# qiqiqicheng/news-recommendation-tc

Hardware: AMD Instinct MI355X
Metric: recalled pairs/sec (YouTubeDNN top-30) + DIN scored pairs/sec, 1/2/4/8 MI355X (higher is better)
Workload: dtype fp16

## Files before the change

### news-recommendation-tc_amd/csrc/ip_topk.hip

```cpp
#include "nrk_common.h"

#include <float.h>
#include <math.h>
#include <stdlib.h>

#include <algorithm>
#include <atomic>
#include <type_traits>
#include <utility>

namespace nrk {

typedef float f32x16 __attribute__((ext_vector_type(16)));
typedef _Float16 f16x8 __attribute__((ext_vector_type(8)));
typedef unsigned u32x4 __attribute__((ext_vector_type(4)));
typedef float f32x4 __attribute__((ext_vector_type(4)));

constexpr int IP_KFAST = 128;
constexpr int IP_KMAX = 2048;
constexpr int SCAN_TILE = 8192;
constexpr int SCAN_TB128 = 4;
__host__ __device__ constexpr int scan_tb(int dp) {
    return dp == 128 ? SCAN_TB128 : (64 * dp >= SCAN_TILE ? 1 : SCAN_TILE / (64 * dp));
}
constexpr int IP_SEL = 512;
constexpr int IP_BQ = 288;
constexpr int IP_KRING = 256;
constexpr size_t CATALOG_HDR = 256;

__host__ __device__ static inline int pad_dim(int d) {
    return d <= 16 ? 16 : d <= 32 ? 32 : d <= 64 ? 64 : d <= 128 ? 128 : 256;
}
__host__ __device__ static inline int64_t n_blocks_of(int64_t n_items) { return (n_items + 31) / 32; }

struct CatalogHdr {
    float max_norm;
    float max_abs;
    float scale;
    int32_t dim;
    int32_t dp;
    float max_dnorm;
};

__device__ __forceinline__ float pow2_scale(float maxabs) {
    if (!(maxabs > 0.0f)) return 1.0f;
    int e;
    (void)frexpf(maxabs, &e);
    return ldexpf(1.0f, 14 - e);
}

// ... 360 lines not shown
}
__device__ __forceinline__ void pf_wait(u32x4 (&cur)[2]) {
    asm volatile("s_waitcnt lgkmcnt(0)" : "+v"(cur[0]), "+v"(cur[1])::"memory");
}
template <int OFF>
__device__ __forceinline__ void pf_issue_at(uint32_t base, u32x4 (&af)[2]) {
    asm volatile("ds_read_b128 %0, %2 offset:%3\n\tds_read_b128 %1, %2 offset:%4"
                 : "=&v"(af[0]), "=&v"(af[1])
                 : "v"(base), "n"(OFF), "n"(OFF + 1024)
                 : "memory");
}
template <int OFF>
__device__ __forceinline__ void pf_wait_issue_at(u32x4 (&cur)[2], uint32_t base, u32x4 (&nxt)[2]) {
    asm volatile("s_waitcnt lgkmcnt(0)\n\tds_read_b128 %0, %4 offset:%5\n\tds_read_b128 %1, %4 offset:%6"
                 : "=&v"(nxt[0]), "=&v"(nxt[1]), "+v"(cur[0]), "+v"(cur[1])
                 : "v"(base), "n"(OFF), "n"(OFF + 1024)
                 : "memory");
}

template <int DP, int NW, int NSL, int UG, int MT>
__global__ __launch_bounds__(NW * 64, 2) void ip_scan_kernel(
    const float* __restrict__ users, int n_users, const uint8_t* __restrict__ catalog, int n_items, int dim, int k,
    int m2, uint2* __restrict__ app, int32_t* __restrict__ acnt, float4* __restrict__ uinfo, int tile_lo,
    int tile_hi, int n_pre, int pstride, float* __restrict__ bnd, int bnd_m) {
    constexpr int DS = DP / 16;
    constexpr int BLOCK_BYTES = 64 * DP;
    constexpr int TB = scan_tb(DP);
    constexpr int TILE_BYTES = TB * BLOCK_BYTES;
    constexpr int LPT = TILE_BYTES / (NW * 1024);
    static_assert(LPT >= 1 && LPT * NW * 1024 == TILE_BYTES, "tile split");
    static_assert(NSL >= 2, "ring");
    __shared__ __attribute__((aligned(16))) uint8_t smem[NSL * TILE_BYTES];

    const int tid = threadIdx.x;
    const int wave = tid >> 6, lane = tid & 63, h = lane >> 5, q = lane & 31;
    const int ub = blockIdx.x;
    const int ubase = ub * (NW * 32 * UG) + wave * (32 * UG);
#if NRK_SCAN_STAMP
    uint64_t sstp[8] = {0, 0, 0, 0, 0, 0, 0, 0};
    uint64_t t_prev = 0;
#endif

    const int nblk = (n_items + 31) >> 5;
    const int ntile = tile_hi;
    const CatalogHdr* hdr = reinterpret_cast<const CatalogHdr*>(catalog + (size_t)nblk * BLOCK_BYTES);
    const float vmax = hdr->max_norm, sv_scale = hdr->scale, dvmax = hdr->max_dnorm;
    const int jk = (k + 1) / 2 - 1;

    f16x8 ufrag[UG][DS];
    float eps_s[UG], tau[UG];
    float t[UG][MT];
    bool live[UG];
#pragma unroll
    for (int g = 0; g < UG; ++g) {
        const int user = ubase + g * 32 + q;
        float eps, scl;
        scan_user_setup<DS>(users, n_users, dim, user, h, vmax, dvmax, sv_scale, ufrag[g], eps, scl, live[g]);
        eps_s[g] = eps * scl;
        if (h == 0 && user < n_users) uinfo[user] = make_float4(-INFINITY, eps_s[g], scl, eps);
        tau[g] = live[g] ? -FLT_MAX : INFINITY;
#pragma unroll
        for (int i = 0; i < MT; ++i) t[g][i] = (live[g] && i >= MT - 1 - jk) ? -INFINITY : INFINITY;
    }
    uint2* const wapp = app + (size_t)(ub * (NW * 32 * UG) + __builtin_amdgcn_readfirstlane(wave) * (32 * UG)) *
                                  2 * (size_t)m2;
    uint32_t pos[UG], lim[UG];
#pragma unroll
    for (int g = 0; g < UG; ++g) {
        pos[g] = (uint32_t)((g * 32 + q) * 2 + h) * (uint32_t)m2;
        lim[g] = pos[g] + (uint32_t)m2 - 1u;
    }
    auto slot = [&](uint32_t x, int g) -> uint32_t { return min(x, lim[g]); };
    auto app_store_if = [&](uint64_t m, uint32_t e, uint2 v) { app_store_masked(m, wapp, e << 3, v); };

    const uint32_t lds_base = (uint32_t)(uintptr_t)(const __attribute__((address_space(3))) uint8_t*)(smem);
    const int body_bytes = nblk * BLOCK_BYTES;
    const int tail_blk = n_items >> 5;
    const int last_tile = (nblk - 1) / TB;
    auto issue_tile = [&](int tt, int sl) {
        uint8_t* slot = smem + sl * TILE_BYTES;
        const uint32_t ttc = (uint32_t)min(tt, last_tile);
#pragma unroll
// ... 256 lines not shown
            if (h == 0) reinterpret_cast<float*>(uinfo + user)[0] = live[g] ? lb : -INFINITY;
        }
    }
    if constexpr (MT <= 32) {
        if (bnd != nullptr) {
#pragma unroll
            for (int g = 0; g < UG; ++g)
                list_bound_out<MT>(t[g], live[g], h, ubase + g * 32 + q, n_users, jk, bnd, bnd_m, uinfo);
        }
    }
}

constexpr int SCAN_WS_NB = 2;
constexpr int SCAN_WS_TPS = 2;
constexpr int SCAN_WS_PRIO = 2;
constexpr int SCAN_WS_INSP = 8, SCAN_WS_SHARD_INSP = 4;
static_assert((SCAN_WS_INSP & (SCAN_WS_INSP - 1)) == 0 && SCAN_WS_INSP >= SCAN_WS_TPS &&
                  (SCAN_WS_SHARD_INSP & (SCAN_WS_SHARD_INSP - 1)) == 0 && SCAN_WS_SHARD_INSP >= SCAN_WS_TPS,
              "insert periods: powers of two >= the two tiles of a step");
template <int DP, int NSL, int MT>
__global__ __launch_bounds__(64 * 4 * (1 + SCAN_WS_NB), 1) void ip_scan_ws_kernel(
    const float* __restrict__ users, int n_users, const uint8_t* __restrict__ catalog, int n_items, int dim, int k,
    int m2, uint2* __restrict__ app, int32_t* __restrict__ acnt, float4* __restrict__ uinfo, int tile_lo,
    int tile_hi, int n_pre, int pstride, float* __restrict__ bnd, int bnd_m, int insp) {
    constexpr int NPW = 4, UG = 8, NB = SCAN_WS_NB, UGB = UG / NB, DS = DP / 16;
    constexpr int BLOCK_BYTES = 64 * DP;
    constexpr int TB = scan_tb(DP);
    constexpr int TILE_BYTES = TB * BLOCK_BYTES;
    constexpr int NPC = TILE_BYTES / 1024;
    static_assert(TB == 4 && DS == 2 && NPC == 8 && UGB == 4, "WS scan: 8-KB tiles of four blocks at DP = 32");
    constexpr int TPS = SCAN_WS_TPS, NMX = 2 * TPS, LPW = NPC / NPW, DAHEAD = NSL / TPS - 1;
    static_assert(NSL % TPS == 0 && DAHEAD >= 1, "ring of whole steps, one step ahead at least");
    constexpr int MXP = TB * 2 * 1024, MXS = NPW * MXP;
    __shared__ __attribute__((aligned(16))) uint8_t smem[NSL * TILE_BYTES];
    __shared__ __attribute__((aligned(16))) uint8_t mxb[NMX * MXS];

    const int tid = threadIdx.x;
    const int wave = tid >> 6, lane = tid & 63, h = lane >> 5, q = lane & 31;
    const int wv = __builtin_amdgcn_readfirstlane(wave);
    const bool mfma_role = wv < NPW;
    const int pw = wv & (NPW - 1);
    const int ubase = (int)blockIdx.x * (NPW * UG * 32) + pw * (UG * 32);
#if NRK_SCAN_STAMP
    uint64_t sstp[8] = {0, 0, 0, 0, 0, 0, 0, 0};
    uint64_t t_prev = __builtin_readcyclecounter();
    auto stamp_out = [&]() {
        if ((threadIdx.x == 0 || threadIdx.x == SCAN_WS_STAMPW * 64) && blockIdx.x < 1024)
// ... 210 lines not shown
        SC_STAMP(0);
#pragma unroll
        for (int j = 0; j < SPC; ++j) dma(j);
        SC_STAMP(1);
        asm volatile("s_waitcnt vmcnt(0)" ::: "memory");
#if NRK_SCAN_STAMP
        SC_STAMP(2);
        stamp_out();
#endif
        return;
    }

    const int gb = ((wv - NPW) / NPW) * UGB;
    float eps_s[UGB], tau[UGB];
    float t[UGB][MT];
    bool live[UGB];
#pragma unroll
    for (int g = 0; g < UGB; ++g) {
        f16x8 uf[DS];
        float eps, scl;
        const int user = ubase + (gb + g) * 32 + q;
        scan_user_setup<DS>(users, n_users, dim, user, h, vmax, dvmax, sv_scale, uf, eps, scl, live[g]);
        eps_s[g] = eps * scl;
        if (h == 0 && user < n_users) uinfo[user] = make_float4(-INFINITY, eps_s[g], scl, eps);
        tau[g] = live[g] ? -FLT_MAX : INFINITY;
#pragma unroll
        for (int i = 0; i < MT; ++i) t[g][i] = (live[g] && i >= MT - 1 - jk) ? -INFINITY : INFINITY;
    }
    uint2* const wapp = app + (size_t)(ubase + gb * 32) * 2 * (size_t)m2;
    const uint32_t off0 = ((uint32_t)(q * 2 + h) * (uint32_t)m2) << 3;
    const size_t gstride = 64u * (size_t)m2;
    uint32_t cnt[UGB];
#pragma unroll
    for (int g = 0; g < UGB; ++g) cnt[g] = 0u;
    auto app_store_if = [&](uint64_t m, int g, uint32_t e, uint2 v) {
        app_store_masked(m, wapp + (size_t)g * gstride, (min(e, (uint32_t)m2 - 1u) << 3) + off0, v);
    };
    auto retau = [&](int g) { tau[g] = scan_tau(t[g][MT - 1], eps_s[g], live[g]); };
    int next_s = n_pre > 0 ? tile_lo : INT_MAX, left_s = n_pre;
#if NRK_SCAN_STAMP
    t_prev = __builtin_readcyclecounter();
#endif
    const uint32_t mq = mx_base + (uint32_t)(gb / 4) * 1024u;
    f32x4 rr[TPS][TB][UGB / 4];
    auto read_issue = [&](int t, uint32_t a) {
        asm volatile(
            "ds_read_b128 %0, %4 offset:0\n\tds_read_b128 %1, %4 offset:2048\n\t"
// ... 287 lines not shown
}

constexpr int SH_WG_PER_CU = 6;
constexpr int SH_ENT = 4;

__device__ __forceinline__ void sh_load(const uint2* s0, const uint2* s1, int a0, int n, int b0, int lane,
                                        uint2 (&ent)[SH_ENT]) {
#pragma unroll
    for (int j = 0; j < SH_ENT; ++j) {
        const int e = b0 + j * WAVE + lane;
        ent[j] = e < n ? (e < a0 ? s0[e] : s1[e - a0]) : make_uint2(0u, 0u);
    }
}

__global__ __launch_bounds__(256) void ip_select_kernel(
    int64_t n_users, int k, int m2, int bandcap, const uint2* __restrict__ app,
    const int32_t* __restrict__ acnt, const float4* __restrict__ uinfo, uint2* __restrict__ cand,
    int32_t* __restrict__ cand_cnt, float2* __restrict__ ucut, int32_t* __restrict__ ovf_flag,
    int32_t* __restrict__ ovf_list, int32_t* __restrict__ ovf_count) {
    __shared__ __attribute__((aligned(16))) uint32_t sel[4][IP_SEL + 4];
    const int lane = threadIdx.x & 63, wave = threadIdx.x >> 6;
    const int64_t nw = (int64_t)gridDim.x * 4;
    const unsigned long long lt = (1ull << lane) - 1ull;
    int64_t u = (int64_t)blockIdx.x * 4 + wave;
    int2 ac_n = make_int2(0, 0);
    float4 inf_n = make_float4(0.f, 0.f, 0.f, 0.f);
    if (u < n_users) {
        ac_n = reinterpret_cast<const int2*>(acnt)[u];
        inf_n = uinfo[u];
    }
    for (; u < n_users; u += nw) {
        const int a0 = ac_n.x, a1 = ac_n.y;
        const float4 inf = inf_n;
        if (u + nw < n_users) {
            ac_n = reinterpret_cast<const int2*>(acnt)[u + nw];
            inf_n = uinfo[u + nw];
        }
        bool ovf = a0 > m2 || a1 > m2;
        const int n = ovf ? 0 : a0 + a1;
        const uint2* s0 = app + (size_t)(2 * u) * m2;
        const uint2* s1 = s0 + m2;
        auto sh_load = [&](int n_, int b0, int lane_, uint2 (&ent)[SH_ENT]) {
#pragma unroll
            for (int j = 0; j < SH_ENT; ++j) {
                const int e = b0 + j * WAVE + lane_;
                const uint2* src = e < a0 ? s0 + e : s1 + (e - a0);
// ... 38 lines not shown
                if (kp && pos < bandcap) bd[pos] = ent[j];
                nb += __popcll(bal);
            }
        }
        if (nb > bandcap) ovf = true;
        if (lane == 0) {
            cand_cnt[u] = ovf ? 0 : nb;
            ucut[u] = make_float2(cut == -INFINITY ? -INFINITY : cut / inf.z, inf.w);
            ovf_flag[u] = ovf ? 1 : 0;
            if (ovf) ovf_list[atomicAdd(ovf_count, 1)] = (int32_t)u;
        }
    }
}

__global__ void ip_all_exact_kernel(int64_t n_users, int32_t* __restrict__ cand_cnt,
                                    int32_t* __restrict__ ovf_flag, int32_t* __restrict__ ovf_list,
                                    int32_t* __restrict__ ovf_count) {
    for (int64_t u = blockIdx.x * (int64_t)blockDim.x + threadIdx.x; u < n_users;
         u += (int64_t)gridDim.x * blockDim.x) {
        cand_cnt[u] = 0;
        ovf_flag[u] = 1;
        ovf_list[u] = (int32_t)u;
    }
    if (blockIdx.x == 0 && threadIdx.x == 0) *ovf_count = (int32_t)n_users;
}

__device__ __forceinline__ double exact_dot(const float* __restrict__ a, const float* __restrict__ b,
                                            int dim) {
    double s = 0.0;
    if ((dim & 31) == 0) {
        const float4* a4 = reinterpret_cast<const float4*>(a);
        const float4* b4 = reinterpret_cast<const float4*>(b);
        for (int t0 = 0; t0 < dim / 4; t0 += 8) {
            float4 x[8], y[8];
#pragma unroll
            for (int t = 0; t < 8; ++t) {
                x[t] = a4[t0 + t];
                y[t] = b4[t0 + t];
            }
#pragma unroll
            for (int t = 0; t < 8; ++t) {
                s += (double)x[t].x * (double)y[t].x;
                s += (double)x[t].y * (double)y[t].y;
                s += (double)x[t].z * (double)y[t].z;
                s += (double)x[t].w * (double)y[t].w;
            }
        }
// ... 2 lines not shown
        const float4* b4 = reinterpret_cast<const float4*>(b);
        for (int t = 0; t < dim / 4; ++t) {
            const float4 x = a4[t], y = b4[t];
            s += (double)x.x * (double)y.x;
            s += (double)x.y * (double)y.y;
            s += (double)x.z * (double)y.z;
            s += (double)x.w * (double)y.w;
        }
    } else {
        for (int t = 0; t < dim; ++t) s += (double)a[t] * (double)b[t];
    }
    return s + 0.0;
}

__device__ __forceinline__ int ring_push(int32_t* ring, int kc, int lane, bool keep, int32_t v) {
    const unsigned long long bal = __ballot(keep);
    if (keep) ring[(kc + __popcll(bal & ((1ull << lane) - 1ull))) & (IP_KRING - 1)] = v;
    kc += __popcll(bal);
    wave_sync_lds();
    return kc;
}

constexpr int REFINE_WPE = 6;
template <int DS4, int SV, bool FK>
__global__ __launch_bounds__(256) __attribute__((amdgpu_waves_per_eu(DS4 == 16 ? 2 : DS4 == 0 ? 4 : REFINE_WPE))) void ip_refine_kernel(
    const float* __restrict__ users, int64_t n_users, const float* __restrict__ items,
    const uint8_t* __restrict__ catalog, int64_t n_items, int dim, int k, int64_t row_offset,
    const uint2* __restrict__ cand, int bandcap, const int32_t* __restrict__ cand_cnt,
    const float2* __restrict__ ucut, const int32_t* __restrict__ ovf_flag, int32_t* __restrict__ ovf_list,
    int32_t* __restrict__ ovf_count, float* __restrict__ out_s, int32_t* __restrict__ out_r,
    double* __restrict__ out_e, int n_src = 0,
    int64_t src_users = 0, int x_cap = 0, const int32_t* __restrict__ src_cnt = nullptr) {
    constexpr int SE = SV / WAVE;
    __shared__ Cand surv[4][SV];
    __shared__ int32_t krow[4][IP_KRING];
    constexpr int RS = DS4 + 1;
    __shared__ float4 stage[DS4 > 0 ? 4 : 1][DS4 > 0 ? 32 * RS : 1];
    __shared__ uint32_t bandq[4][SV + 32 > IP_BQ ? SV + 32 : IP_BQ];
    __shared__ __attribute__((aligned(16))) float ushl[4][DS4 > 0 ? 1 : 256];
    const int lane = threadIdx.x & 63, wave = threadIdx.x >> 6;
    const int64_t u = (int64_t)blockIdx.x * 4 + wave;
    if (u >= n_users) return;
    const bool slots = n_src == 0;
    const float* uv = users + u * dim;
    const int32_t ovf_u = ovf_flag[u];
    const int nbd_slots = slots ? cand_cnt[u] : 0;
    const float2 ce = ucut[u];
    const float uv_r = uv[lane < dim ? lane : 0];
    const uint2 ent0 = slots ? cand[(size_t)u * bandcap + (lane < 32 ? lane : 0)] : make_uint2(0u, 0u);
    if (ovf_u) return;
    int src_n = 0;
    int nsrc_tot = 0;
    if (n_src > 0) {
        for (int s0 = 0; s0 < n_src; s0 += WAVE) {
            const int sl = s0 + lane;
            const int c = sl < n_src ? max(0, src_cnt[(int64_t)sl * src_users + u]) : 0;
            if (s0 == 0) src_n = c;
            nsrc_tot += (int)wave_sum_f32((float)c);
        }
    }
    if (nsrc_tot > IP_BQ) {
        if ((threadIdx.x & 63) == 0) ovf_list[atomicAdd(ovf_count, 1)] = (int32_t)u;
        return;
    }
    const float uv_l = lane < dim ? uv_r : 0.0f;
    float nz = fabsf(uv_l), uam = fabsf(uv_l);
    for (int d = lane + WAVE; d < dim; d += WAVE) {
        nz += fabsf(uv[d]);
        uam = fmaxf(uam, fabsf(uv[d]));
    }
    nz = wave_sum_f32(nz);
    if (nz == 0.0f) {
        for (int i = lane; i < k; i += WAVE) {
            const bool ok = i < n_items;
            out_s[u * k + i] = ok ? 0.0f : -FLT_MAX;
            out_r[u * k + i] = ok ? (int32_t)(i + row_offset) : -1;
            if (out_e) out_e[u * k + i] = ok ? 0.0 : -INFINITY;
        }
        return;
    }
    const int nbd = n_src > 0 ? 0 : nbd_slots;
    const uint2* bd = cand + (size_t)u * bandcap;
    double thr = -INFINITY;
    if (ce.x != -INFINITY) {
        thr = (double)ce.x + (double)ce.y;
        thr = thr - fabs(thr) * 1e-15 - 1e-300;
    }
    constexpr int DSK = DS4 / 4;
    const bool pre = catalog != nullptr && ce.x != -INFINITY;
    __shared__ __attribute__((aligned(16))) _Float16 ushs[4][DS4 > 0 ? 4 * DS4 : 8];
    _Float16* ush = ushs[wave];
    float pcut = 0.0f;
    if (pre) {
        const int dpc = pad_dim(dim);
        const int64_t nblk_c = (n_items + 31) >> 5;
        const CatalogHdr* hdr = reinterpret_cast<const CatalogHdr*>(catalog + (size_t)nblk_c * 64 * dpc);
        float ua = uam;
#pragma unroll
        for (int m = 32; m > 0; m >>= 1) ua = fmaxf(ua, __shfl_xor(ua, m, WAVE));
        const float su = pow2_scale(ua);
        if constexpr (DS4 > 0) {
#pragma unroll
            for (int d = lane; d < 4 * DS4; d += WAVE) ush[d] = (_Float16)(uv[d] * su);
            wave_sync_lds();
        }
        pcut = ce.x * (su * hdr->scale);
    }
    int nband = 0;
    auto take_one = [&](uint2 ent, int e, int cnt) {
        const bool kp = e < cnt && (!pre || __uint_as_float(ent.x) >= pcut);
        const unsigned long long bal = __ballot(kp);
        if (kp) bandq[wave][nband + __popcll(bal & ((1ull << lane) - 1ull))] = ent.y;
        nband += __popcll(bal);
    };
    auto take = [&](const uint2* __restrict__ src, int cnt) {
        int b0 = 0;
        if (slots) {
            take_one(ent0, lane < 32 ? lane : cnt, cnt);
            b0 = 32;
        }
        for (; b0 < cnt; b0 += WAVE) {
            const int e = b0 + lane;
            take_one(e < cnt ? src[e] : make_uint2(0u, 0u), e, cnt);
        }
    };
    if (n_src > 0) {
        const uint32_t* ids = reinterpret_cast<const uint32_t*>(cand);
        for (int s2 = 0; s2 < n_src; ++s2) {
            const int c2 = s2 < WAVE ? __shfl(src_n, s2, WAVE) : max(0, src_cnt[(int64_t)s2 * src_users + u]);
            const uint32_t* src = ids + ((size_t)s2 * src_users + u) * x_cap;
            for (int b0 = 0; b0 < c2; b0 += WAVE) {
                const int e = b0 + lane;
                if (e < c2) bandq[wave][nband + e] = src[e];
                nband += min(WAVE, c2 - b0);
            }
        }
    } else {
        take(bd, nbd);
    }
    wave_sync_lds();
    const int nitem = nband * 16;
    int cnt = 0;
    auto push = [&](bool keep, double s, int32_t row) {
        const unsigned long long bal = __ballot(keep);
        const int pos = cnt + __popcll(bal & ((1ull << lane) - 1ull));
        if (keep && pos < SV) surv[wave][pos] = Cand{s, row};
        cnt += __popcll(bal);
    };
    if constexpr (DS4 > 0) {
        constexpr bool LANES = DS4 == 4 || DS4 == 8;
        const uint8_t* hbc = catalog ? catalog + catalog_hb_offset(n_items, 4 * DS4) : nullptr;
        int kc = 0, ko = 0;
        auto exact_round = [&](int m) {
            int32_t rl = lane < m ? krow[wave][(ko + lane) & (IP_KRING - 1)] : -1;
            if constexpr (LANES) {
                if (rl >= 0) {
                    const uint32_t qv = bandq[wave][rl >> 4];
                    const int r = rl & 15;
// ... 224 lines not shown
                    float acc = 0.0f;
                    for (int st = 0; st < dskc; ++st) {
                        const f16x8 h0 = __builtin_bit_cast(f16x8, *reinterpret_cast<const uint4*>(bp + st * 1024 + il * 16));
                        const f16x8 h1 =
                            __builtin_bit_cast(f16x8, *reinterpret_cast<const uint4*>(bp + st * 1024 + (il + 32) * 16));
                        const float* us = &ushl[wave][16 * st];
#pragma unroll
                        for (int e = 0; e < 8; ++e) acc = fmaf((float)h0[e], us[e], acc);
#pragma unroll
                        for (int e = 0; e < 8; ++e) acc = fmaf((float)h1[e], us[8 + e], acc);
                    }
                    keep = acc >= pcut;
                }
            }
            const unsigned long long bal = __ballot(keep);
            if (keep) krow[wave][(kc + __popcll(bal & ((1ull << lane) - 1ull))) & (IP_KRING - 1)] = row;
            kc += __popcll(bal);
            wave_sync_lds();
            while (kc - ko >= WAVE) exact_generic(WAVE);
        }
        while (kc > ko) exact_generic(kc - ko < WAVE ? kc - ko : WAVE);
    }
    if (cnt > SV) {
        if (lane == 0) ovf_list[atomicAdd(ovf_count, 1)] = (int32_t)u;
        return;
    }
    wave_sync_lds();
    auto emit = [&](const Cand* x, int ne) {
        for (int e = 0; e < ne; ++e) {
            const int idx = e * 64 + lane;
            if (idx < k) {
                const bool ok = x[e].row != INT32_MAX;
                out_s[u * k + idx] = ok ? (float)x[e].s : -FLT_MAX;
                out_r[u * k + idx] = ok ? (int32_t)(x[e].row + row_offset) : -1;
                if (out_e) out_e[u * k + idx] = ok ? x[e].s : -INFINITY;
            }
        }
    };
    if (SE > 1 && cnt <= WAVE && k <= WAVE) {
        if constexpr (FK) {
            uint64_t key = 0;
            if (lane < cnt) {
                const Cand c = surv[wave][lane];
                key = ((uint64_t)fkey((float)c.s) << 32) | (uint32_t)~c.row;
            }
            key = wave_sort_desc_u64(key);
            const uint32_t hi = (uint32_t)(key >> 32);
// ... 16 lines not shown
    }
    Cand x[SE];
#pragma unroll
    for (int e = 0; e < SE; ++e) {
        const int idx = e * 64 + lane;
        if (idx < cnt) x[e] = surv[wave][idx];
        else { x[e].s = -INFINITY; x[e].row = INT32_MAX; }
    }
    wave_bitonic_sort<SE>(x);
    emit(x, SE);
}

__device__ __forceinline__ uint64_t okey(double s) {
    const uint64_t b = (uint64_t)__double_as_longlong(s);
    return (b >> 63) ? ~b : (b | 0x8000000000000000ull);
}

constexpr int FB_GRID = 256;

__global__ __launch_bounds__(256) void ip_exact_kernel(
    const float* __restrict__ users, const float* __restrict__ items, int64_t n_items, int dim, int k, int ns,
    int64_t row_offset, const int32_t* __restrict__ ovf_list, const int32_t* __restrict__ ovf_count,
    float* __restrict__ out_s, int32_t* __restrict__ out_r, double* __restrict__ out_e,
    uint32_t* __restrict__ scratch, int32_t* __restrict__ slow_list, int32_t* __restrict__ slow_count) {
    extern __shared__ __attribute__((aligned(16))) uint8_t dyn[];
    Cand* sel = reinterpret_cast<Cand*>(dyn);
    __shared__ unsigned int hist[2048];
    __shared__ unsigned int part[256];
    __shared__ int s_bin, s_krem, s_eq, sel_n;
    const int tid = threadIdx.x, lane = tid & 63;
    const int cnt = *ovf_count;
    const int kk = (int)(n_items < k ? n_items : k);
    uint32_t* key = scratch + (size_t)blockIdx.x * n_items;
    for (int qi = blockIdx.x; qi < cnt; qi += gridDim.x) {
        const int64_t u = ovf_list[qi];
        const float* uv = users + u * dim;
        for (int64_t r = tid; r < n_items; r += 256) key[r] = fkey((float)exact_dot(uv, items + r * dim, dim));
        __syncthreads();
        uint32_t prefix = 0, mask = 0;
        int krem = kk;
        for (int p = 0; p < 3; ++p) {
            const int wbits = p < 2 ? 11 : 10, sh = p == 0 ? 21 : (p == 1 ? 10 : 0);
            const uint32_t nbm = (1u << wbits) - 1u;
            for (int i = tid; i < 2048; i += 256) hist[i] = 0u;
            __syncthreads();
            for (int64_t r0 = 0; r0 < n_items; r0 += 256) {
                const int64_t r = r0 + tid;
                const uint32_t kv = r < n_items ? key[r] : 0u;
                const bool act = r < n_items && (kv & mask) == prefix;
                const uint32_t b = (kv >> sh) & nbm;
                unsigned long long pend = __ballot(act);
                while (pend) {
                    const int l = __ffsll((long long)pend) - 1;
                    const uint32_t bl = (uint32_t)__shfl((int)b, l, WAVE);
// ... 55 lines not shown
                    const Cand a = sel[lo], b = sel[hi];
                    if (up ? better(b, a) : better(a, b)) {
                        sel[lo] = b;
                        sel[hi] = a;
                    }
                }
                __syncthreads();
            }
        }
        for (int i = tid; i < k; i += 256) {
            const bool ok = i < kk;
            out_s[u * k + i] = ok ? (float)sel[i].s : -FLT_MAX;
            out_r[u * k + i] = ok ? (int32_t)(sel[i].row + row_offset) : -1;
            if (out_e) out_e[u * k + i] = ok ? sel[i].s : -INFINITY;
        }
        __syncthreads();
    }
}

__global__ __launch_bounds__(256) void ip_fallback_kernel(
    const float* __restrict__ users, const float* __restrict__ items, int64_t n_items, int dim,
    int k, int ns, int64_t row_offset, const int32_t* __restrict__ ovf_list,
    const int32_t* __restrict__ ovf_count, float* __restrict__ out_s, int32_t* __restrict__ out_r,
    double* __restrict__ out_e) {
    extern __shared__ __attribute__((aligned(16))) uint8_t dyn[];
    Cand* sel = reinterpret_cast<Cand*>(dyn);
    __shared__ unsigned int hist[256];
    __shared__ int sel_n;
    __shared__ unsigned long long s_prefix;
    __shared__ int s_krem;
    __shared__ int wcnt[4];
    const int tid = threadIdx.x, lane = tid & 63, wave = tid >> 6;
    const int cnt = *ovf_count;
    const int kk = (int)(n_items < k ? n_items : k);
    for (int qi = blockIdx.x; qi < cnt; qi += gridDim.x) {
        const int64_t u = ovf_list[qi];
        const float* uv = users + u * dim;
        unsigned long long prefix = 0, mask = 0;
        int krem = kk;
        for (int pass = 7; pass >= 0 && kk > 0; --pass) {
            hist[tid] = 0;
            __syncthreads();
            for (int64_t r = tid; r < n_items; r += 256) {
                const uint64_t key = okey(exact_dot(uv, items + r * dim, dim));
                if ((key & mask) == prefix) atomicAdd(&hist[(key >> (8 * pass)) & 255], 1u);
            }
            __syncthreads();
            if (tid == 0) {
                int cum = 0, b = 255;
                for (; b > 0; --b) {
                    if (cum + (int)hist[b] >= krem) break;
                    cum += hist[b];
                }
                s_prefix = prefix | ((unsigned long long)b << (8 * pass));
                s_krem = krem - cum;
            }
// ... 423 lines not shown
struct ScanRange {
    int t_lo, t_hi, n_pre, pstride;
};
static ScanRange scan_range(int tb, int n_items, const IpWs& w) {
    const int nblk = (n_items + 31) / 32;
    ScanRange r;
    r.t_lo = w.blk_lo / tb;
    r.t_hi = (std::min(w.blk_hi, nblk) + tb - 1) / tb;
    const int n = r.t_hi - r.t_lo;
    const int pre_div = w.bnd != nullptr ? SCAN_SHARD_PRE_DIV : SCAN_PRE_DIV;
    r.n_pre = n >= SCAN_PRE_MIN ? std::min(SCAN_PRE_MAX, n / pre_div) : 0;
    r.pstride = r.n_pre > 0 ? n / r.n_pre : 1;
    return r;
}

template <int DP, int NW, int NSL, int UG, int MT>
static void launch_scan_v(const float* users, int n_users, const uint8_t* cat, int n_items, int dim, int k,
                          const IpWs& w, hipStream_t s) {
    const int per_wg = NW * 32 * UG;
    const ScanRange r = scan_range(scan_tb(DP), n_items, w);
    const unsigned grid = (unsigned)((n_users + per_wg - 1) / per_wg);
    ip_scan_kernel<DP, NW, NSL, UG, MT><<<grid, NW * 64, 0, s>>>(
        users, n_users, cat, n_items, dim, k, w.m2, w.app, w.acnt, w.uinfo, r.t_lo, r.t_hi, r.n_pre, r.pstride,
        w.bnd, w.bnd_m);
}

constexpr int SCAN_NSL4 = 4;
constexpr int SCAN128_NSL = 4;
template <int DP, int MT>
static void launch_scan(const float* users, int n_users, const uint8_t* cat, int n_items, int dim, int k,
                        const IpWs& w, hipStream_t s) {
    if constexpr (DP == 32 && MT == 16) {
        const int per_wg = 4 * 8 * 32;
        const ScanRange r = scan_range(scan_tb(DP), n_items, w);
        const unsigned grid = (unsigned)((n_users + per_wg - 1) / per_wg);
        const int insp = w.bnd != nullptr ? SCAN_WS_SHARD_INSP : SCAN_WS_INSP;
        ip_scan_ws_kernel<DP, SCAN_NSL4, MT><<<grid, 256 * (1 + SCAN_WS_NB), 0, s>>>(
            users, n_users, cat, n_items, dim, k, w.m2, w.app, w.acnt, w.uinfo, r.t_lo, r.t_hi, r.n_pre, r.pstride,
            w.bnd, w.bnd_m, insp);
    } else {
        constexpr int UG = (DP <= 128 && MT <= 32) ? 2 : 1;
        constexpr int TILE_B = scan_tb(DP) * 64 * DP, NSL_CAP = 163840 / TILE_B;
        constexpr int NW = (UG == 2) ? 8 : 4, NSL0 = (UG == 2) ? (DP == 128 ? SCAN128_NSL : 3) : 4,
                      NSL = NSL0 < NSL_CAP ? NSL0 : NSL_CAP;
        static_assert(NSL >= 2, "ring");
        launch_scan_v<DP, NW, NSL, UG, MT>(users, n_users, cat, n_items, dim, k, w, s);
    }
}

template <int DP>
static void launch_scan_k(const float* users, int n_users, const uint8_t* cat, int n_items, int dim, int k,
                          const IpWs& w, hipStream_t s) {
    const int mt = (k + 1) / 2;
    if (mt <= 16) launch_scan<DP, 16>(users, n_users, cat, n_items, dim, k, w, s);
    else if (mt <= 32) launch_scan<DP, 32>(users, n_users, cat, n_items, dim, k, w, s);
    else launch_scan<DP, 64>(users, n_users, cat, n_items, dim, k, w, s);
}

static void scan_dispatch(const float* users, int nu, const uint8_t* cat, int ni, int dim, int k, const IpWs& w,
                          hipStream_t s) {
    switch (pad_dim(dim)) {
        case 16: launch_scan_k<16>(users, nu, cat, ni, dim, k, w, s); break;
// ... 21 lines not shown
}

__global__ void ip_empty_range_kernel(int64_t n_users, int32_t* __restrict__ acnt, float4* __restrict__ uinfo) {
    for (int64_t u = blockIdx.x * (int64_t)blockDim.x + threadIdx.x; u < n_users;
         u += (int64_t)gridDim.x * blockDim.x) {
        acnt[2 * u] = 0;
        acnt[2 * u + 1] = 0;
        uinfo[u] = make_float4(-INFINITY, 0.0f, 0.0f, 0.0f);
    }
}

static void launch_exact(const float* users, int64_t n_users, const float* items, int64_t n_items, int dim, int k,
                         int64_t row_offset, const IpWs& w, float* out_s, int32_t* out_r, double* out_e,
                         hipStream_t s) {
    const int ns = pow2_at_least(k, 64);
    const size_t lds = (size_t)ns * sizeof(Cand);
    constexpr size_t lds_max = pow2_at_least(IP_KMAX) * sizeof(Cand);
    static_assert(lds_max <= CU_LDS_BYTES, "ip_exact / ip_fallback LDS");
    static std::atomic<uint64_t> exact_set{0}, fallback_set{0};
    lds_limit_once(exact_set, (const void*)ip_exact_kernel, lds_max);
    lds_limit_once(fallback_set, (const void*)ip_fallback_kernel, lds_max);
    const int grid = (int)std::min<int64_t>(n_users, FB_GRID);
    ip_exact_kernel<<<grid, 256, lds, s>>>(users, items, n_items, dim, k, ns, row_offset, w.ovf_list, w.ovf_count,
                                           out_s, out_r, out_e, w.fbk, w.slow_list, w.ovf_count + 1);
    ip_fallback_kernel<<<grid, 256, lds, s>>>(users, items, n_items, dim, k, ns, row_offset, w.slow_list,
                                              w.ovf_count + 1, out_s, out_r, out_e);
}

template <class F>
static void with_sort_width(int total, F&& fn) {
    if (total <= 64) fn(std::integral_constant<int, 1>{}, 64);
    else if (total <= 128) fn(std::integral_constant<int, 2>{}, 128);
    else if (total <= 256) fn(std::integral_constant<int, 4>{}, 256);
    else fn(std::integral_constant<int, 0>{}, pow2_at_least(total));
}
template <int E>
static size_t sort_lds_bytes(int ns) {
    return E ? 0 : 4 * (size_t)ns * sizeof(Cand);
}

struct RefineBand {
    const uint2* cand;
    int bandcap;
    const int32_t* cnt;
    const float2* ucut;
    int n_src = 0;
    int64_t src_users = 0;
    int x_cap = 0;
    const int32_t* src_cnt = nullptr;
};

static void launch_refine(const float* users, int64_t n_users, const float* items, const uint8_t* cat, int64_t n_items,
                          int dim, int k, int64_t row_offset, const RefineBand& b, const IpWs& w, float* out_s,
                          int32_t* out_r, double* out_e, hipStream_t s) {
    const int g2 = (int)((n_users + 3) / 4);
    auto go = [&](auto ds4, auto sv, auto fk) {
        ip_refine_kernel<decltype(ds4)::value, decltype(sv)::value, decltype(fk)::value><<<g2, 256, 0, s>>>(
            users, n_users, items, cat, n_items, dim, k, row_offset, b.cand, b.bandcap, b.cnt, b.ucut, w.ovf_flag,
            w.ovf_list, w.ovf_count, out_s, out_r, out_e, b.n_src, b.src_users, b.x_cap, b.src_cnt);
    };
    auto by_sv = [&](auto ds4) {
        if (k > 64) go(ds4, std::integral_constant<int, 256>{}, std::false_type{});
        else if (out_e) go(ds4, std::integral_constant<int, 128>{}, std::false_type{});
        else go(ds4, std::integral_constant<int, 128>{}, std::true_type{});
    };
    if (dim == 32) by_sv(std::integral_constant<int, 8>{});
    else if (dim == 16) by_sv(std::integral_constant<int, 4>{});
    else if (dim == 64) by_sv(std::integral_constant<int, 16>{});
    else by_sv(std::integral_constant<int, 0>{});
}

}

using namespace nrk;

extern "C" {

#if NRK_SCAN_STAMP
int nrk_dev_scan_stamps(unsigned long long* out) {
    return hipMemcpyFromSymbol(out, HIP_SYMBOL(scan_stamps), sizeof(scan_stamps)) == hipSuccess ? 0 : -1;
}
#endif
// ... 65 lines not shown
}

static int screen_phases(const float* users, int64_t n_users, const void* catalog, int64_t n_items, int dim, int k,
                         int64_t blk_lo, int64_t blk_hi, void* workspace, size_t workspace_bytes,
                         nrk_stream_t stream, int phases) {
    int rc = ip_check(users, n_users, (const float*)catalog, catalog, n_items, dim, k, workspace,
                      workspace_bytes);
    if (rc != NRK_OK || n_users == 0) return rc;
    IpWs w = ip_ws_layout(workspace, n_users, n_items, k, dim);
    rc = ip_range(w, n_items, dim, blk_lo, blk_hi);
    if (rc != NRK_OK) return rc;
    if (blk_hi == blk_lo) n_items = 0;
    hipStream_t s = as_stream(stream);
    const uint8_t* cat = reinterpret_cast<const uint8_t*>(catalog);
    if ((phases & 1) && n_items > 0 && k <= IP_KFAST) {
        scan_dispatch(users, (int)n_users, cat, (int)n_items, dim, k, w, s);
    }
    if (phases & 2) {
        NRK_FILL("nrk_ip_topk_screen", w.ovf_count, 0, 256, s);
        if (n_items == 0) {
            (void)hipMemsetAsync(w.cnt, 0, (size_t)n_users * sizeof(int32_t), s);
            (void)hipMemsetAsync(w.ovf_flag, 0, (size_t)n_users * sizeof(int32_t), s);
            (void)hipMemsetAsync(w.ucut, 0xFF, (size_t)n_users * sizeof(float2), s);
        } else if (k > IP_KFAST) {
            ip_all_exact_kernel<<<grid_for(n_users, 256, 4096), 256, 0, s>>>(n_users, w.cnt, w.ovf_flag, w.ovf_list,
                                                                             w.ovf_count);
        } else {
            ip_select_kernel<<<sh_grid(n_users), 256, 0, s>>>(n_users, k, w.m2, w.bandcap, w.app, w.acnt, w.uinfo,
                                                              w.cand, w.cnt, w.ucut, w.ovf_flag, w.ovf_list,
                                                              w.ovf_count);
        }
    }
    NRK_CHECK_LAUNCH();
    return NRK_OK;
}

int nrk_ip_topk_scan(const float* users, int64_t n_users, const void* catalog, int64_t n_items, int dim, int k,
                     void* workspace, size_t workspace_bytes, nrk_stream_t stream) {
    clear_error();
    return screen_phases(users, n_users, catalog, n_items, dim, k, 0, n_blocks_of(n_items), workspace,
                         workspace_bytes, stream, 1);
}

int nrk_ip_topk_select(const float* users, int64_t n_users, const void* catalog, int64_t n_items, int dim, int k,
                       void* workspace, size_t workspace_bytes, nrk_stream_t stream) {
    clear_error();
    return screen_phases(users, n_users, catalog, n_items, dim, k, 0, n_blocks_of(n_items), workspace,
                         workspace_bytes, stream, 2);
}

int nrk_ip_topk_screen(const float* users, int64_t n_users, const void* catalog, int64_t n_items,
                       int dim, int k, void* workspace, size_t workspace_bytes,
                       nrk_stream_t stream) {
// ... 28 lines not shown
                nrk_stream_t stream) {
    int rc = nrk_ip_topk_screen(users, n_users, catalog, n_items, dim, k, workspace,
                                workspace_bytes, stream);
    if (rc != NRK_OK) return rc;
    return nrk_ip_topk_finish(users, n_users, items, catalog, n_items, dim, k, row_offset, out_scores,
                              out_rows, out_exact, workspace, workspace_bytes, stream);
}

int nrk_ip_topk_bound(const float* users, int64_t n_users, const void* catalog, int64_t n_items, int dim,
                      int k, int m, float* out_bound, void* workspace, size_t workspace_bytes,
                      nrk_stream_t stream) {
    clear_error();
    int rc = ip_check(users, n_users, (const float*)catalog, catalog, n_items, dim, k, workspace,
                      workspace_bytes);
    if (rc != NRK_OK) return rc;
    if (k > IP_KFAST) NRK_UNSUPPORTED("the screen bound needs k <= 128");
    NRK_REQUIRE(m >= 1 && m <= 256, "m must be in [1, 256]");
    if (n_users == 0) return NRK_OK;
    NRK_REQUIRE(out_bound != nullptr, "null pointer");
    const IpWs w = ip_ws_layout(workspace, n_users, n_items, k, dim);
    hipStream_t s = as_stream(stream);
    if (n_items == 0) {
        (void)hipMemsetAsync(w.cnt, 0, (size_t)n_users * sizeof(int32_t), s);
    }
    const CatalogHdr* hdr = reinterpret_cast<const CatalogHdr*>(
        reinterpret_cast<const uint8_t*>(catalog) + catalog_body_bytes(n_items, pad_dim(dim)));
    const int grid = (int)((n_users + 3) / 4);
    with_sort_width(std::max(w.bandcap, m), [&](auto ec, int ns) {
        constexpr int E = decltype(ec)::value;
        ip_bound_kernel<E><<<grid, 256, sort_lds_bytes<E>(ns), s>>>(users, n_users, dim, hdr, w.cand, w.bandcap, w.cnt,
                                                                    w.ucut, m, ns, out_bound);
    });
    NRK_CHECK_LAUNCH();
    return NRK_OK;
}

int nrk_ip_topk_apply_bound(int64_t n_users, const float* bounds, int n_lists, int m, int k, void* workspace,
                            size_t workspace_bytes, nrk_stream_t stream) {
    clear_error();
    NRK_REQUIRE(n_users >= 0 && n_users < (1ll << 30), "n_users out of range");
    NRK_REQUIRE(n_lists >= 1 && m >= 1 && n_lists * m <= 512, "need 1 <= n_lists * m <= 512");
    NRK_REQUIRE(k >= 1 && k <= IP_KFAST, "k must be in [1, 128]");
    if (n_users == 0) return NRK_OK;
    NRK_REQUIRE(bounds && workspace, "null pointer");
    NRK_REQUIRE(workspace_bytes >= ip_ws_layout(nullptr, n_users, 0, 1, 1).bytes, "workspace too small");
    const IpWs w = ip_ws_layout(workspace, n_users, 0, 1, 1);
// ... 120 lines not shown
```

Baseline: 1.299 billion.

## Fuse band selection into refine kernel by reading scan append lists directly

Removes the separate ip_select kernel from the default screen path and has the refine kernel read the per-user append lists, counts and uinfo directly, doing the band cut and a k-th-key tightening in-wave. A device flag in the overflow counter array records whether the band buffers were built. In that case refine takes the old slot path; the bound path still launches select itself. This saves a kernel launch and the round trip through the candidate buffer, but adds list reads and an LDS select inside refine. Overflow pushes are now capped at n_users.

```diff
diff --git a/news-recommendation-tc_amd/csrc/ip_topk.hip b/news-recommendation-tc_amd/csrc/ip_topk.hip
--- a/news-recommendation-tc_amd/csrc/ip_topk.hip
+++ b/news-recommendation-tc_amd/csrc/ip_topk.hip
@@ -26,6 +26,7 @@
 constexpr int IP_SEL = 512;
 constexpr int IP_BQ = 288;
 constexpr int IP_KRING = 256;
+constexpr int WS_BAND_BUILT = 2;
 constexpr size_t CATALOG_HDR = 256;
 
 __host__ __device__ static inline int pad_dim(int d) {
@@ -432,7 +433,7 @@
 __global__ __launch_bounds__(NW * 64, 2) void ip_scan_kernel(
     const float* __restrict__ users, int n_users, const uint8_t* __restrict__ catalog, int n_items, int dim, int k,
     int m2, uint2* __restrict__ app, int32_t* __restrict__ acnt, float4* __restrict__ uinfo, int tile_lo,
-    int tile_hi, int n_pre, int pstride, float* __restrict__ bnd, int bnd_m) {
+    int tile_hi, int n_pre, int pstride, float* __restrict__ bnd, int bnd_m, float2* __restrict__ ucut) {
     constexpr int DS = DP / 16;
     constexpr int BLOCK_BYTES = 64 * DP;
     constexpr int TB = scan_tb(DP);
@@ -467,7 +468,10 @@
         float eps, scl;
         scan_user_setup<DS>(users, n_users, dim, user, h, vmax, dvmax, sv_scale, ufrag[g], eps, scl, live[g]);
         eps_s[g] = eps * scl;
-        if (h == 0 && user < n_users) uinfo[user] = make_float4(-INFINITY, eps_s[g], scl, eps);
+        if (h == 0 && user < n_users) {
+            uinfo[user] = make_float4(-INFINITY, eps_s[g], scl, eps);
+            ucut[user] = make_float2(-INFINITY, eps);
+        }
         tau[g] = live[g] ? -FLT_MAX : INFINITY;
 #pragma unroll
         for (int i = 0; i < MT; ++i) t[g][i] = (live[g] && i >= MT - 1 - jk) ? -INFINITY : INFINITY;
@@ -770,7 +774,7 @@
 __global__ __launch_bounds__(64 * 4 * (1 + SCAN_WS_NB), 1) void ip_scan_ws_kernel(
     const float* __restrict__ users, int n_users, const uint8_t* __restrict__ catalog, int n_items, int dim, int k,
     int m2, uint2* __restrict__ app, int32_t* __restrict__ acnt, float4* __restrict__ uinfo, int tile_lo,
-    int tile_hi, int n_pre, int pstride, float* __restrict__ bnd, int bnd_m, int insp) {
+    int tile_hi, int n_pre, int pstride, float* __restrict__ bnd, int bnd_m, int insp, float2* __restrict__ ucut) {
     constexpr int NPW = 4, UG = 8, NB = SCAN_WS_NB, UGB = UG / NB, DS = DP / 16;
     constexpr int BLOCK_BYTES = 64 * DP;
     constexpr int TB = scan_tb(DP);
@@ -1027,7 +1031,10 @@
         const int user = ubase + (gb + g) * 32 + q;
         scan_user_setup<DS>(users, n_users, dim, user, h, vmax, dvmax, sv_scale, uf, eps, scl, live[g]);
         eps_s[g] = eps * scl;
-        if (h == 0 && user < n_users) uinfo[user] = make_float4(-INFINITY, eps_s[g], scl, eps);
+        if (h == 0 && user < n_users) {
+            uinfo[user] = make_float4(-INFINITY, eps_s[g], scl, eps);
+            ucut[user] = make_float2(-INFINITY, eps);
+        }
         tau[g] = live[g] ? -FLT_MAX : INFINITY;
 #pragma unroll
         for (int i = 0; i < MT; ++i) t[g][i] = (live[g] && i >= MT - 1 - jk) ? -INFINITY : INFINITY;
@@ -1361,6 +1368,7 @@
     const int lane = threadIdx.x & 63, wave = threadIdx.x >> 6;
     const int64_t nw = (int64_t)gridDim.x * 4;
     const unsigned long long lt = (1ull << lane) - 1ull;
+    if (blockIdx.x == 0 && threadIdx.x == 0) ovf_count[WS_BAND_BUILT] = 1;
     int64_t u = (int64_t)blockIdx.x * 4 + wave;
     int2 ac_n = make_int2(0, 0);
     float4 inf_n = make_float4(0.f, 0.f, 0.f, 0.f);
@@ -1445,7 +1453,10 @@
         ovf_flag[u] = 1;
         ovf_list[u] = (int32_t)u;
     }
-    if (blockIdx.x == 0 && threadIdx.x == 0) *ovf_count = (int32_t)n_users;
+    if (blockIdx.x == 0 && threadIdx.x == 0) {
+        *ovf_count = (int32_t)n_users;
+        ovf_count[WS_BAND_BUILT] = 1;
+    }
 }
 
 __device__ __forceinline__ double exact_dot(const float* __restrict__ a, const float* __restrict__ b,
@@ -1494,32 +1505,72 @@
 }
 
 constexpr int REFINE_WPE = 6;
+constexpr int REFINE_LW = 128;
+__device__ __forceinline__ void ovf_push(int32_t* __restrict__ ovf_list, int32_t* __restrict__ ovf_count,
+                                         int64_t n_users, int64_t u) {
+    const int p = atomicAdd(ovf_count, 1);
+    if (p < n_users) ovf_list[p] = (int32_t)u;
+}
 template <int DS4, int SV, bool FK>
 __global__ __launch_bounds__(256) __attribute__((amdgpu_waves_per_eu(DS4 == 16 ? 2 : DS4 == 0 ? 4 : REFINE_WPE))) void ip_refine_kernel(
     const float* __restrict__ users, int64_t n_users, const float* __restrict__ items,
     const uint8_t* __restrict__ catalog, int64_t n_items, int dim, int k, int64_t row_offset,
     const uint2* __restrict__ cand, int bandcap, const int32_t* __restrict__ cand_cnt,
     const float2* __restrict__ ucut, const int32_t* __restrict__ ovf_flag, int32_t* __restrict__ ovf_list,
-    int32_t* __restrict__ ovf_count, float* __restrict__ out_s, int32_t* __restrict__ out_r,
-    double* __restrict__ out_e, int n_src = 0,
+    int32_t* __restrict__ ovf_count, const int32_t* __restrict__ band_built, const uint2* __restrict__ app, int m2,
+    const int32_t* __restrict__ acnt, const float4* __restrict__ uinfo, float* __restrict__ out_s,
+    int32_t* __restrict__ out_r, double* __restrict__ out_e, int n_src = 0,
     int64_t src_users = 0, int x_cap = 0, const int32_t* __restrict__ src_cnt = nullptr) {
     constexpr int SE = SV / WAVE;
     __shared__ Cand surv[4][SV];
     __shared__ int32_t krow[4][IP_KRING];
     constexpr int RS = DS4 + 1;
     __shared__ float4 stage[DS4 > 0 ? 4 : 1][DS4 > 0 ? 32 * RS : 1];
-    __shared__ uint32_t bandq[4][SV + 32 > IP_BQ ? SV + 32 : IP_BQ];
+    constexpr int BQN = SV + 32 > IP_BQ ? SV + 32 : IP_BQ;
+    __shared__ uint32_t bandq[4][BQN];
     __shared__ __attribute__((aligned(16))) float ushl[4][DS4 > 0 ? 1 : 256];
     const int lane = threadIdx.x & 63, wave = threadIdx.x >> 6;
     const int64_t u = (int64_t)blockIdx.x * 4 + wave;
     if (u >= n_users) return;
     const bool slots = n_src == 0;
+    const bool lists = slots && *band_built == 0;
     const float* uv = users + u * dim;
-    const int32_t ovf_u = ovf_flag[u];
-    const int nbd_slots = slots ? cand_cnt[u] : 0;
-    const float2 ce = ucut[u];
     const float uv_r = uv[lane < dim ? lane : 0];
-    const uint2 ent0 = slots ? cand[(size_t)u * bandcap + (lane < 32 ? lane : 0)] : make_uint2(0u, 0u);
+    int32_t ovf_u = 0;
+    int nbd_slots = 0;
+    float2 ce = make_float2(-INFINITY, 0.0f);
+    float cut_s = -INFINITY;
+    float eps_sc = 0.0f, scl = 1.0f;
+    int2 ac = make_int2(0, 0);
+    constexpr int LWN = REFINE_LW / WAVE;
+    uint2 lw[2][LWN] = {};
+    if (lists) {
+        const uint2* l0 = app + (size_t)(2 * u) * m2;
+        ac = reinterpret_cast<const int2*>(acnt)[u];
+        const float4 ui = uinfo[u];
+#pragma unroll
+        for (int w = 0; w < 2; ++w)
+#pragma unroll
+            for (int j = 0; j < LWN; ++j) lw[w][j] = l0[(size_t)w * m2 + min(j * WAVE + lane, m2 - 1)];
+        if (ac.x > m2 || ac.y > m2) {
+            if (lane == 0) ovf_push(ovf_list, ovf_count, n_users, u);
+            return;
+        }
+        eps_sc = ui.y;
+        scl = ui.z;
+        if (ui.x != -INFINITY) {
+            cut_s = round_down_sub(ui.x, 2.0f * ui.y);
+            ce = make_float2(cut_s / ui.z, ui.w);
+        } else {
+            ce.y = ui.w;
+        }
+    } else {
+        ovf_u = ovf_flag[u];
+        nbd_slots = slots ? cand_cnt[u] : 0;
+        ce = ucut[u];
+        if (slots) lw[0][0] = cand[(size_t)u * bandcap + (lane < 32 ? lane : 0)];
+    }
+    const uint2 ent0 = lw[0][0];
     if (ovf_u) return;
     int src_n = 0;
     int nsrc_tot = 0;
@@ -1532,7 +1583,7 @@
         }
     }
     if (nsrc_tot > IP_BQ) {
-        if ((threadIdx.x & 63) == 0) ovf_list[atomicAdd(ovf_count, 1)] = (int32_t)u;
+        if (lane == 0) ovf_push(ovf_list, ovf_count, n_users, u);
         return;
     }
     const float uv_l = lane < dim ? uv_r : 0.0f;
@@ -1553,16 +1604,18 @@
     }
     const int nbd = n_src > 0 ? 0 : nbd_slots;
     const uint2* bd = cand + (size_t)u * bandcap;
+    auto cut_thr = [](float cx, float eps) {
+        const double t = (double)cx + (double)eps;
+        return t - fabs(t) * 1e-15 - 1e-300;
+    };
     double thr = -INFINITY;
-    if (ce.x != -INFINITY) {
-        thr = (double)ce.x + (double)ce.y;
-        thr = thr - fabs(thr) * 1e-15 - 1e-300;
-    }
+    if (ce.x != -INFINITY) thr = cut_thr(ce.x, ce.y);
     constexpr int DSK = DS4 / 4;
     const bool pre = catalog != nullptr && ce.x != -INFINITY;
+    const bool bcut = lists ? ce.x != -INFINITY : pre;
     __shared__ __attribute__((aligned(16))) _Float16 ushs[4][DS4 > 0 ? 4 * DS4 : 8];
     _Float16* ush = ushs[wave];
-    float pcut = 0.0f;
+    float pcut = cut_s;
     if (pre) {
         const int dpc = pad_dim(dim);
         const int64_t nblk_c = (n_items + 31) >> 5;
@@ -1576,13 +1629,15 @@
             for (int d = lane; d < 4 * DS4; d += WAVE) ush[d] = (_Float16)(uv[d] * su);
             wave_sync_lds();
         }
-        pcut = ce.x * (su * hdr->scale);
+        if (!lists) pcut = ce.x * (su * hdr->scale);
     }
     int nband = 0;
     auto take_one = [&](uint2 ent, int e, int cnt) {
-        const bool kp = e < cnt && (!pre || __uint_as_float(ent.x) >= pcut);
+        const bool kp = e < cnt && (!bcut || __uint_as_float(ent.x) >= pcut);
         const unsigned long long bal = __ballot(kp);
-        if (kp) bandq[wave][nband + __popcll(bal & ((1ull << lane) - 1ull))] = ent.y;
+        const int pos = nband + __popcll(bal & ((1ull << lane) - 1ull));
+        if (kp && pos < BQN) bandq[wave][pos] = ent.y;
+        if (lists && kp && pos < WAVE) krow[wave][pos] = (int32_t)fkey(__uint_as_float(ent.x));
         nband += __popcll(bal);
     };
     auto take = [&](const uint2* __restrict__ src, int cnt) {
@@ -1606,6 +1661,36 @@
                 if (e < c2) bandq[wave][nband + e] = src[e];
                 nband += min(WAVE, c2 - b0);
             }
+        }
+    } else if (lists) {
+#pragma unroll
+        for (int w = 0; w < 2; ++w) {
+            const int a = w ? ac.y : ac.x;
+            const uint2* src = app + (size_t)(2 * u + w) * m2;
+#pragma unroll
+            for (int j = 0; j < LWN; ++j)
+                if (j * WAVE < a) take_one(lw[w][j], j * WAVE + lane, a);
+            for (int b0 = REFINE_LW; b0 < a; b0 += WAVE) {
+                const int e = b0 + lane;
+                take_one(e < a ? src[e] : make_uint2(0u, 0u), e, a);
+            }
+        }
+        if (nband > BQN) {
+            if (lane == 0) ovf_push(ovf_list, ovf_count, n_users, u);
+            return;
+        }
+        if (bcut && nband <= WAVE && nband >= k) {
+            const float theta = fkey_inv(lds_select(reinterpret_cast<uint32_t*>(krow[wave]), nband, k - 1, lane));
+            const float cut2 = round_down_sub(theta, 2.0f * eps_sc);
+            const uint32_t key = lane < nband ? (uint32_t)krow[wave][lane] : 0u;
+            const uint32_t id = bandq[wave][lane < nband ? lane : 0];
+            const bool kp = lane < nband && fkey_inv(key) >= cut2;
+            const unsigned long long bal = __ballot(kp);
+            wave_sync_lds();
+            if (kp) bandq[wave][__popcll(bal & ((1ull << lane) - 1ull))] = id;
+            nband = __popcll(bal);
+            pcut = cut2;
+            thr = cut_thr(cut2 / scl, ce.y);
         }
     } else {
         take(bd, nbd);
@@ -1876,7 +1961,7 @@
         while (kc > ko) exact_generic(kc - ko < WAVE ? kc - ko : WAVE);
     }
     if (cnt > SV) {
-        if (lane == 0) ovf_list[atomicAdd(ovf_count, 1)] = (int32_t)u;
+        if (lane == 0) ovf_push(ovf_list, ovf_count, n_users, u);
         return;
     }
     wave_sync_lds();
@@ -1939,14 +2024,15 @@
     const float* __restrict__ users, const float* __restrict__ items, int64_t n_items, int dim, int k, int ns,
     int64_t row_offset, const int32_t* __restrict__ ovf_list, const int32_t* __restrict__ ovf_count,
     float* __restrict__ out_s, int32_t* __restrict__ out_r, double* __restrict__ out_e,
-    uint32_t* __restrict__ scratch, int32_t* __restrict__ slow_list, int32_t* __restrict__ slow_count) {
+    uint32_t* __restrict__ scratch, int32_t* __restrict__ slow_list, int32_t* __restrict__ slow_count,
+    int list_cap) {
     extern __shared__ __attribute__((aligned(16))) uint8_t dyn[];
     Cand* sel = reinterpret_cast<Cand*>(dyn);
     __shared__ unsigned int hist[2048];
     __shared__ unsigned int part[256];
     __shared__ int s_bin, s_krem, s_eq, sel_n;
     const int tid = threadIdx.x, lane = tid & 63;
-    const int cnt = *ovf_count;
+    const int cnt = min(*ovf_count, list_cap);
     const int kk = (int)(n_items < k ? n_items : k);
     uint32_t* key = scratch + (size_t)blockIdx.x * n_items;
     for (int qi = blockIdx.x; qi < cnt; qi += gridDim.x) {
@@ -2048,7 +2134,7 @@
     const float* __restrict__ users, const float* __restrict__ items, int64_t n_items, int dim,
     int k, int ns, int64_t row_offset, const int32_t* __restrict__ ovf_list,
     const int32_t* __restrict__ ovf_count, float* __restrict__ out_s, int32_t* __restrict__ out_r,
-    double* __restrict__ out_e) {
+    double* __restrict__ out_e, int list_cap) {
     extern __shared__ __attribute__((aligned(16))) uint8_t dyn[];
     Cand* sel = reinterpret_cast<Cand*>(dyn);
     __shared__ unsigned int hist[256];
@@ -2057,7 +2143,7 @@
     __shared__ int s_krem;
     __shared__ int wcnt[4];
     const int tid = threadIdx.x, lane = tid & 63, wave = tid >> 6;
-    const int cnt = *ovf_count;
+    const int cnt = min(*ovf_count, list_cap);
     const int kk = (int)(n_items < k ? n_items : k);
     for (int qi = blockIdx.x; qi < cnt; qi += gridDim.x) {
         const int64_t u = ovf_list[qi];
@@ -2527,7 +2613,7 @@
     const unsigned grid = (unsigned)((n_users + per_wg - 1) / per_wg);
     ip_scan_kernel<DP, NW, NSL, UG, MT><<<grid, NW * 64, 0, s>>>(
         users, n_users, cat, n_items, dim, k, w.m2, w.app, w.acnt, w.uinfo, r.t_lo, r.t_hi, r.n_pre, r.pstride,
-        w.bnd, w.bnd_m);
+        w.bnd, w.bnd_m, w.ucut);
 }
 
 constexpr int SCAN_NSL4 = 4;
@@ -2542,7 +2628,7 @@
         const int insp = w.bnd != nullptr ? SCAN_WS_SHARD_INSP : SCAN_WS_INSP;
         ip_scan_ws_kernel<DP, SCAN_NSL4, MT><<<grid, 256 * (1 + SCAN_WS_NB), 0, s>>>(
             users, n_users, cat, n_items, dim, k, w.m2, w.app, w.acnt, w.uinfo, r.t_lo, r.t_hi, r.n_pre, r.pstride,
-            w.bnd, w.bnd_m, insp);
+            w.bnd, w.bnd_m, insp, w.ucut);
     } else {
         constexpr int UG = (DP <= 128 && MT <= 32) ? 2 : 1;
         constexpr int TILE_B = scan_tb(DP) * 64 * DP, NSL_CAP = 163840 / TILE_B;
@@ -2610,9 +2696,9 @@
     lds_limit_once(fallback_set, (const void*)ip_fallback_kernel, lds_max);
     const int grid = (int)std::min<int64_t>(n_users, FB_GRID);
     ip_exact_kernel<<<grid, 256, lds, s>>>(users, items, n_items, dim, k, ns, row_offset, w.ovf_list, w.ovf_count,
-                                           out_s, out_r, out_e, w.fbk, w.slow_list, w.ovf_count + 1);
+                                           out_s, out_r, out_e, w.fbk, w.slow_list, w.ovf_count + 1, (int)n_users);
     ip_fallback_kernel<<<grid, 256, lds, s>>>(users, items, n_items, dim, k, ns, row_offset, w.slow_list,
-                                              w.ovf_count + 1, out_s, out_r, out_e);
+                                              w.ovf_count + 1, out_s, out_r, out_e, (int)n_users);
 }
 
 template <class F>
@@ -2645,7 +2731,8 @@
     auto go = [&](auto ds4, auto sv, auto fk) {
         ip_refine_kernel<decltype(ds4)::value, decltype(sv)::value, decltype(fk)::value><<<g2, 256, 0, s>>>(
             users, n_users, items, cat, n_items, dim, k, row_offset, b.cand, b.bandcap, b.cnt, b.ucut, w.ovf_flag,
-            w.ovf_list, w.ovf_count, out_s, out_r, out_e, b.n_src, b.src_users, b.x_cap, b.src_cnt);
+            w.ovf_list, w.ovf_count, w.ovf_count + WS_BAND_BUILT, w.app, w.m2, w.acnt, w.uinfo, out_s, out_r, out_e,
+            b.n_src, b.src_users, b.x_cap, b.src_cnt);
     };
     auto by_sv = [&](auto ds4) {
         if (k > 64) go(ds4, std::integral_constant<int, 256>{}, std::false_type{});
@@ -2757,13 +2844,10 @@
             (void)hipMemsetAsync(w.cnt, 0, (size_t)n_users * sizeof(int32_t), s);
             (void)hipMemsetAsync(w.ovf_flag, 0, (size_t)n_users * sizeof(int32_t), s);
             (void)hipMemsetAsync(w.ucut, 0xFF, (size_t)n_users * sizeof(float2), s);
+            (void)hipMemsetD32Async(reinterpret_cast<hipDeviceptr_t>(w.ovf_count + WS_BAND_BUILT), 1, 1, s);
         } else if (k > IP_KFAST) {
             ip_all_exact_kernel<<<grid_for(n_users, 256, 4096), 256, 0, s>>>(n_users, w.cnt, w.ovf_flag, w.ovf_list,
                                                                              w.ovf_count);
-        } else {
-            ip_select_kernel<<<sh_grid(n_users), 256, 0, s>>>(n_users, k, w.m2, w.bandcap, w.app, w.acnt, w.uinfo,
-                                                              w.cand, w.cnt, w.ucut, w.ovf_flag, w.ovf_list,
-                                                              w.ovf_count);
         }
     }
     NRK_CHECK_LAUNCH();
@@ -2838,6 +2922,10 @@
     hipStream_t s = as_stream(stream);
     if (n_items == 0) {
         (void)hipMemsetAsync(w.cnt, 0, (size_t)n_users * sizeof(int32_t), s);
+    } else {
+        NRK_FILL(__func__, w.ovf_count, 0, 256, s);
+        ip_select_kernel<<<sh_grid(n_users), 256, 0, s>>>(n_users, k, w.m2, w.bandcap, w.app, w.acnt, w.uinfo, w.cand,
+                                                          w.cnt, w.ucut, w.ovf_flag, w.ovf_list, w.ovf_count);
     }
     const CatalogHdr* hdr = reinterpret_cast<const CatalogHdr*>(
         reinterpret_cast<const uint8_t*>(catalog) + catalog_body_bytes(n_items, pad_dim(dim)));
```

New measurement: 1.327 billion, median of 6. 1.02x the previous value.
